# JinfengX/PointCloudPDF

Hardware: AMD Instinct MI355X
Metric: points/sec fwd+bwd (PT-v1 Seg50 + PDF U-decoder, 100k-pt scenes) (higher is better)
Workload: dtype f32

## Files before the change

### include/pdfops.h

```cpp
#ifndef PDFOPS_H
#define PDFOPS_H

#ifdef __cplusplus
extern "C" {
#endif

#define PDF_OK 0
#define PDF_ERR_BAD_ARG (-1)
#define PDF_ERR_NSAMPLE (-2)
#define PDF_ERR_UNSUPPORTED (-3)

#define PDF_ABI_VERSION 7
int pdf_abi_version(void);
const char *pdf_build_info(void);
int pdf_dist_fma_mode(void);
#define PDF_MMA_F32 0
#define PDF_MMA_F16 1
#define PDF_MMA_BF16 2

int pdf_knn_query(int m, int nsample, const float *xyz, const float *new_xyz,
                  const int *offset, const int *new_offset, int b,
                  int *idx, float *dist2, void *stream);

long pdf_knn_workspace_bytes(int b, int n, int m);
int pdf_knn_grid_supported(int nsample);
int pdf_knn_query_ws(int m, int nsample, int n, const float *xyz, const float *new_xyz, const int *offset,
                     const int *new_offset, int b, int *idx, float *dist2, void *workspace, long workspace_bytes,
                     void *stream);
int pdf_knn_grid_build(int n, const float *xyz, const int *offset, int b, void *workspace, long workspace_bytes, void *stream);
int pdf_knn_query_grid(int m, int nsample, int n, const float *xyz, const float *new_xyz, const int *offset, const int *new_offset, int b,
                       int *idx, float *dist2, void *workspace, long workspace_bytes, void *stream);
int pdf_knn_query_ws_counted(int m, int nsample, int n, const float *xyz, const float *new_xyz, const int *offset,
                             const int *new_offset, int b, int *idx, float *dist2, void *workspace, long workspace_bytes,
                             unsigned long long *pairs, void *stream);
int pdf_knn_query_list(int m, int nsample, const float *xyz, const float *new_xyz, const int *offset,
// ... 119 lines not shown
                      const float *k_points, float extent, float *weighted, void *stream);
int pdf_kpconv_scatter(int n, int m, int kp, int cin, const float *query, const float *support, const int *neighbors,
                       const float *grad_weighted, const float *k_points, float extent, float *grad_x, void *stream);
int pdf_rowlin_dgrad_bstats(long n, int k, int o, int nin, const float *const *x, long ldx, const float *const *w, float *y, long ldy,
                            const float *bx, long ldb, const float *bcoef, int brelu, float *partial, int *partial_rows,
                            int mma_input, void *stream);
int pdf_rowlin_forward_bn(long n, int k, int o, const float *x, long ldx, const float *w, const float *bias, const float *scale,
                          const float *shift, int relu, float *y, long ldy, float *partial, const float *gamma, const float *beta,
                          float *running_mean, float *running_var, float eps, float momentum, float *coef, int mma_input, void *stream);
int pdf_bn_act_backward_presummed(long n, int c, const float *gy, const float *x, const float *coef, int training, int relu,
                                  const float *partial, int partial_rows, float *sums, float *gx, void *stream);

int pdf_bn_coef_eval_or_partial(const float *partial, int rows, long n, int c, const float *gamma, const float *beta,
                                float *running_mean, float *running_var, int training, float eps, float momentum,
                                float *coef, void *stream);
int pdf_block_pre_forward(long n, int c, void *const *p, int training, float eps, float momentum, int mma_input, void *stream);
int pdf_block_pre_backward(long n, int c, void *const *p, int training, int mma_input, void *stream);
int pdf_block_post_forward(long n, int c, void *const *p, int training, float eps, float momentum, int mma_input, void *stream);
int pdf_block_post_backward(long n, int c, void *const *p, int training, int mma_input, void *stream);
int pdf_bottleneck_forward(long n, int nsample, int c, void *const *p, int training, float eps, float momentum, int storage_bf16, int mma_input, void *stream);
int pdf_bottleneck_backward(long n, int nsample, int c, void *const *p, int training, int entry_base, int storage_bf16, int mma_input, void *stream);
int pdf_linbn_forward(long n, int k, int o, void *const *p, int training, int relu, float eps, float momentum, int mma_input, void *stream);
int pdf_linbn_backward(long n, int k, int o, void *const *p, int training, int relu, int mma_input, void *stream);

int pdf_rowlin_forward_roww(long n, int k, int o, const float *x, long ldx, const float *w, int transpose_w, float *y, long ldy,
                            int accumulate, const float *roww, long rws, int mma_input, void *stream);
int pdf_rowlin_wgrad_roww(long n, int k, int o, const float *g, long ldg, const float *x, long ldx, float *dw, const float *roww,
                          long rws, float *ws, int mma_input, void *stream);
int pdf_bn_bwd_sums(long n, int c, const float *gy, const float *x, const float *coef, int relu, float *partial, float *sums,
                    void *stream);

int pdf_td_supported(int nsample, int cin, int cout);
int pdf_td_tables(long m, int b, const float *p_src, const float *p_new, const int *idx, const int *new_offset, float *rel4, float *Z,
                  float *scene_sums, long n, const int *inv_off, const int *inv_entry, int entry_base,
                  void *stream);
long pdf_td_gram_floats(int cin);
long pdf_td_fwd_scratch_floats(long n, int cin);
long pdf_td_bwd_scratch_floats(long m, int cin, int cout);
int pdf_td_forward(long n, long m, int cin, int cout, void *const *p, int training, float eps, float momentum, int mma_input, void *stream);
int pdf_td_backward(long n, long m, int cin, int cout, void *const *p, int entry_base, int mma_input, void *stream);

int pdf_seg_sum_rows(long n, int c, const float *src, const int *inv_off, const int *inv_entry, int entry_base, float scale, float *out,
                     void *stream);
int pdf_seg_sum_rows_own(long n, int c, int nsample, const float *src, const int *inv_off, const int *inv_entry, int entry_base, float scale,
                         const int *order, float *out, float *out_own, void *stream);
int pdf_seg_sum_rows_strided(long n, int c, const float *src, long src_stride, const int *inv_off, const int *inv_entry, int entry_base,
// ... 183 lines not shown
```

### pointcloudpdf_amd/_native.py

```python
import ctypes
import os
import threading

import torch

_HERE = os.path.dirname(os.path.abspath(__file__))
DIST_FMA = int(os.environ.get("PDFOPS_DIST_FMA", "0") or 0)
if DIST_FMA not in (0, 1, 2):
    raise RuntimeError(f"PDFOPS_DIST_FMA={DIST_FMA}: expected 0 (as written), 1 or 2 (csrc/pdfops_common.h)")


def library_path(dist_fma=0):
    return os.path.join(_HERE, "lib", "libpdfops.so" if not dist_fma else f"libpdfops_fma{int(dist_fma)}.so")


LIB_PATH = library_path(DIST_FMA)
ABI_VERSION = 7

c_int = ctypes.c_int
c_long = ctypes.c_long
c_void_p = ctypes.c_void_p
c_float = ctypes.c_float
c_double = ctypes.c_double

_PROTOS = {
    "knn_query": "iippppipp",
    "ball_query": "iiffppppipp",
    "random_ball_query": "iiffpppppipp",
    "farthest_point_sampling": "iippppp",
    "grouping_forward": "iiippp",
    "grouping_backward": "iiippp",
    "interpolation_forward": "iiipppp",
    "interpolation_backward": "iiipppp",
    "subtraction_forward": "iiipppp",
    "subtraction_backward": "iiipppp",
    "aggregation_forward": "iiiippppp",
    "aggregation_backward": "iiiipppppppp",
    "attention_relation_step_forward": "iiipppppp",
    "attention_relation_step_backward": "iiippppppppp",
    "attention_fusion_step_forward": "iiippppp",
# ... 581 lines not shown

        self.CopySeg = CopySeg
        lib.pdf_stage_copy.restype = c_int
        lib.pdf_stage_copy.argtypes = [c_int, c_void_p, c_void_p]
        lib.pdf_scene_morton_keys.restype = c_int
        lib.pdf_scene_morton_keys.argtypes = [c_long, c_int, c_void_p, c_void_p, c_void_p, c_void_p, c_void_p]
        lib.pdf_sgd_chunk.restype = c_int
        lib.pdf_sgd_chunk.argtypes = []
        lib.pdf_sgd_step.restype = c_int
        lib.pdf_sgd_step.argtypes = [c_int, c_void_p, c_void_p, ctypes.c_float, ctypes.c_float, ctypes.c_float, c_void_p, c_void_p]
        lib.pdf_grad_unscale.restype = c_int
        lib.pdf_grad_unscale.argtypes = [c_int, c_void_p, c_void_p, c_void_p, c_void_p, c_void_p]
        lib.pdf_scaler_update.restype = c_int
        lib.pdf_scaler_update.argtypes = [c_void_p, c_void_p, c_void_p, c_void_p, ctypes.c_float, ctypes.c_float, c_int, c_void_p]
        lib.pdf_adam_step.restype = c_int
        lib.pdf_adam_step.argtypes = [c_int, c_int, c_void_p, c_void_p, ctypes.c_double, ctypes.c_double, ctypes.c_double, ctypes.c_double,
                                      ctypes.c_double, c_int, c_void_p, c_void_p]
        lib.pdf_adam_grad_unscale.restype = c_int
        lib.pdf_adam_grad_unscale.argtypes = [c_int, c_void_p, c_void_p, c_void_p, c_void_p, c_void_p]
        lib.pdf_linbn_forward.restype = c_int
        lib.pdf_linbn_forward.argtypes = [c_long, c_int, c_int, c_void_p, c_int, c_int, ctypes.c_float, ctypes.c_float, c_int, c_void_p]
        lib.pdf_linbn_backward.restype = c_int
        lib.pdf_linbn_backward.argtypes = [c_long, c_int, c_int, c_void_p, c_int, c_int, c_int, c_void_p]
        lib.pdf_bottleneck_forward.restype = c_int
        lib.pdf_bottleneck_forward.argtypes = [c_long, c_int, c_int, c_void_p, c_int, ctypes.c_float, ctypes.c_float, c_int, c_int, c_void_p]
        lib.pdf_bottleneck_backward.restype = c_int
        lib.pdf_bottleneck_backward.argtypes = [c_long, c_int, c_int, c_void_p, c_int, c_int, c_int, c_int, c_void_p]
        for nm in ("pre_backward", "post_backward"):
            f = getattr(lib, "pdf_block_" + nm)
            f.restype = c_int
            f.argtypes = [c_long, c_int, c_void_p, c_int, c_int, c_void_p]
        lib.pdf_rowlin_multi.restype = c_int
        lib.pdf_rowlin_multi.argtypes = [c_long, c_int, c_int, c_int, c_int, c_void_p, c_long, c_void_p, c_int, c_void_p, c_void_p, c_void_p,
                                         c_int, c_void_p, c_long, c_int, c_int, c_void_p]
        lib.pdf_kpconv_supported.restype = c_int
        lib.pdf_kpconv_supported.argtypes = [c_int, c_int]
        for nm in ("pdf_kpconv_gather", "pdf_kpconv_scatter"):
            f = getattr(lib, nm)
            f.restype = c_int
            f.argtypes = [c_int, c_int, c_int, c_int, c_void_p, c_void_p, c_void_p, c_void_p, c_void_p, ctypes.c_float, c_void_p, c_void_p]
        lib.pdf_rowlin_wgrad_group.restype = c_int
        lib.pdf_rowlin_wgrad_group.argtypes = [c_long, c_int, c_int, c_int, c_void_p, c_long, c_void_p, c_long, c_void_p, c_void_p, c_void_p,
                                               c_void_p, c_void_p, c_void_p, c_int, c_void_p]
        lib.pdf_rowlin_wgrad_multi.restype = c_int
        lib.pdf_rowlin_wgrad_multi.argtypes = [c_long, c_int, c_int, c_int, c_void_p, c_long, c_void_p, c_long, c_void_p, c_void_p, c_int,
                                               c_void_p, c_void_p, c_void_p, c_int, c_void_p]
# ... 1026 lines not shown
```

### pointcloudpdf_amd/csrc/block.hip

```cpp
#include "pdfops_common.h"

namespace {
struct Err {
    int rc = 0;
    Err &operator<<(int r) { if (rc == 0 && r != 0) rc = r; return *this; }
};

}

extern "C" int pdf_bn_coef_eval_or_partial(const float *partial, int rows, long n, int c, const float *gamma, const float *beta,
                                           float *running_mean, float *running_var, int training, float eps, float momentum,
                                           float *coef, void *stream) {
    if (training) return pdf_bn_coef_from_partial(partial, rows, n, c, gamma, beta, running_mean, running_var, eps, momentum, coef, stream);
    return pdf_bn_coef(n, c, nullptr, gamma, beta, running_mean, running_var, 0, eps, momentum, coef, nullptr, stream);
}

extern "C" int pdf_block_pre_forward(long n, int c, void *const *p, int training, float eps, float momentum, int mma_input, void *stream) {
    if (n < 1 || !p) return PDF_ERR_BAD_ARG;
    if (!pdf_bn_supported(c)) return PDF_ERR_UNSUPPORTED;
    const float *x = (const float *)p[0], *W1 = (const float *)p[1], *g1 = (const float *)p[2], *b1 = (const float *)p[3];
    float *rm1 = (float *)p[4], *rv1 = (float *)p[5];
    float *z1 = (float *)p[12], *coef1 = (float *)p[13], *partial = (float *)p[17];
    Err e;
    if (training) {
// ... 180 lines not shown
    float *z = (float *)p[7], *coef = (float *)p[8], *partial = (float *)p[10];
    if (training) {
        e << pdf_rowlin_forward_bn(n, k, o, (const float *)p[0], k, (const float *)p[1], (const float *)p[2], nullptr, nullptr, 0, z, o, partial,
                                   (const float *)p[3], (const float *)p[4], (float *)p[5], (float *)p[6], eps, momentum, coef, mma_input, stream);
    } else {
        e << pdf_rowlin_forward(n, k, o, (const float *)p[0], k, (const float *)p[1], 0, (const float *)p[2], nullptr, nullptr, 0, z, o, 0, nullptr, mma_input, stream);
        e << pdf_bn_coef_eval_or_partial(partial, 0, n, o, (const float *)p[3], (const float *)p[4], (float *)p[5], (float *)p[6], 0, eps, momentum, coef, stream);
    }
    e << pdf_bn_apply(n, o, z, nullptr, coef, relu, (float *)p[9], stream);
    return e.rc;
}

extern "C" int pdf_linbn_backward(long n, int k, int o, void *const *p, int training, int relu, int mma_input, void *stream) {
    if (n < 1 || !p || !p[9]) return PDF_ERR_BAD_ARG;
    float *grads = (float *)p[6], *gz = (float *)p[7];
    const long ok = (long)o * k;
    Err e;
    e << pdf_bn_act_backward(n, o, (const float *)p[0], (const float *)p[2], nullptr, (const float *)p[3], training, relu, (float *)p[8],
                             grads + ok + o, gz, nullptr, stream);
    if (p[5]) e << pdf_rowlin_forward(n, o, k, gz, o, (const float *)p[4], 1, nullptr, nullptr, nullptr, 0, (float *)p[5], k, 0, nullptr, mma_input, stream);
    e << pdf_rowlin_wgrad(n, k, o, gz, o, (const float *)p[1], k, nullptr, nullptr, 0, grads, grads + ok, (float *)p[9], mma_input, stream);
    return e.rc;
}
```

### pointcloudpdf_amd/csrc/fused_layer.hip

```cpp
#include "fused_layer.h"
#include <algorithm>
#include <cstdlib>

namespace fl {

__host__ __device__ constexpr int tile_stride(int c) { return c / 8 > 32 ? 65 : 33; }
__host__ __device__ constexpr int aux_stride(int c) { return c / 8 <= 16 ? 17 : c / 8 + 1; }
constexpr int MAX_BLOCKS = 512;
static inline int env_blocks(const char *name, int dflt) {
    const char *v = getenv(name);
    const int x = v ? atoi(v) : 0;
    return x > 0 ? x : dflt;
}

struct WaveLds {
    float *tile;
    float *qtile;
    int *rowid;
    float *aux;
    int ts, as;
};

__device__ __forceinline__ void wave_sync() {
    __builtin_amdgcn_fence(__ATOMIC_RELEASE, "wavefront");
// ... 788 lines not shown
        for (int t = 0; t < RED_B; ++t) v[t] = src[(size_t)min(r + t * RED_RL, rows - 1) * stride];
#pragma unroll
        for (int t = 0; t < RED_B; ++t) v[t] = (r + t * RED_RL < rows) ? v[t] : 0.f;
#pragma unroll
        for (int t = 0; t < RED_B; t += 4) { s0 += (double)v[t]; s1 += (double)v[t + 1]; s2 += (double)v[t + 2]; s3 += (double)v[t + 3]; }
    }
    return (s0 + s1) + (s2 + s3);
}

__device__ __forceinline__ double wave_rows_sum(double v) {
    v += __shfl_xor(v, 16, 64);
    v += __shfl_xor(v, 32, 64);
    return v;
}
constexpr int RED_WAVES = RED_THREADS / 64;

struct BnpClosed {
    const double *mom;
    cfloat_p Wp1, bp1, sp, mean, rstd;
    double rows;
    int col_g;
    float *out4;
};
__global__ __launch_bounds__(RED_THREADS) void k_colsum(const float *__restrict__ partial, int rows, int width, int stride, float *__restrict__ out,
                                                        BnpClosed bc) {
    __shared__ double red[RED_WAVES][17];
    if (blockIdx.x * 16 >= (unsigned)width) {
        __shared__ double col[16];
        const int cl = threadIdx.x & 15, rl = threadIdx.x >> 4;
        const int c = cl < 6 ? cl : bc.col_g + (cl - 6);
        const double v = wave_rows_sum(cl < 15 ? strided_sum(partial + c, (size_t)stride, rl, rows) : 0.0);
        if ((threadIdx.x & 63) < 16) red[threadIdx.x >> 6][cl] = v;
        __syncthreads();
        if (threadIdx.x < 16) {
            double s = 0.0;
#pragma unroll
            for (int k = 0; k < RED_WAVES; ++k) s += red[k][threadIdx.x];
            col[threadIdx.x] = s;
        }
        __syncthreads();
        if (threadIdx.x < 12) {
            const double S[3] = {bc.mom[0], bc.mom[1], bc.mom[2]};
            const double M[3][3] = {{bc.mom[3], bc.mom[4], bc.mom[5]}, {bc.mom[4], bc.mom[6], bc.mom[7]}, {bc.mom[5], bc.mom[7], bc.mom[8]}};
            const int a = threadIdx.x < 3 ? (int)threadIdx.x : ((int)threadIdx.x - 3) / 3, b = threadIdx.x < 3 ? 0 : ((int)threadIdx.x - 3) % 3;
            const double w[3] = {(double)bc.Wp1[a * 3], (double)bc.Wp1[a * 3 + 1], (double)bc.Wp1[a * 3 + 2]};
            const double d = (double)bc.bp1[a] - (double)bc.mean[a], rs = (double)bc.rstd[a], sp = (double)bc.sp[a], R = bc.rows;
            const double s_a = col[a], u_a = col[3 + a];
            double r;
            if (threadIdx.x < 3) {
                const double sum_that = rs * (w[0] * S[0] + w[1] * S[1] + w[2] * S[2] + R * d);
                r = sp * (-(u_a / R) * sum_that);
            } else {
                const double T = rs * (w[0] * M[0][b] + w[1] * M[1][b] + w[2] * M[2][b] + d * S[b]);
                r = sp * (col[6 + 3 * a + b] - s_a * S[b] / R - u_a * T / R);
            }
            bc.out4[threadIdx.x] = (float)r;
        } else if (threadIdx.x < 16) {
            bc.out4[threadIdx.x] = 0.f;
        }
        return;
    }
    const int cl = threadIdx.x & 15, rl = threadIdx.x >> 4;
    const int col = blockIdx.x * 16 + cl;
    const double v = wave_rows_sum(col < width ? strided_sum(partial + col, (size_t)stride, rl, rows) : 0.0);
    if ((threadIdx.x & 63) < 16) red[threadIdx.x >> 6][cl] = v;
    __syncthreads();
    if (rl != 0 || col >= width) return;
    double s = 0.0;
#pragma unroll
    for (int k = 0; k < RED_WAVES; ++k) s += red[k][cl];
    out[col] = (float)s;
}

__global__ __launch_bounds__(RED_THREADS) void k_bn_finalize(const float *__restrict__ partial, int rows, int nch, double count,
                              const float *__restrict__ gamma, const float *__restrict__ beta, float eps, float momentum,
                              float *__restrict__ running_mean, float *__restrict__ running_var,
                              float *__restrict__ scale, float *__restrict__ shift, float *__restrict__ mean_out,
                              float *__restrict__ rstd_out) {
    __shared__ double red[2][RED_WAVES][17];
    const int cl = threadIdx.x & 15, rl = threadIdx.x >> 4;
    const int ch = blockIdx.x * 16 + cl;
    const double a = wave_rows_sum(ch < nch ? strided_sum(partial + ch, 2 * (size_t)nch, rl, rows) : 0.0);
    const double b = wave_rows_sum(ch < nch ? strided_sum(partial + nch + ch, 2 * (size_t)nch, rl, rows) : 0.0);
    if ((threadIdx.x & 63) < 16) { red[0][threadIdx.x >> 6][cl] = a; red[1][threadIdx.x >> 6][cl] = b; }
    __syncthreads();
    if (rl != 0 || ch >= nch) return;
    double s = 0.0, ss = 0.0;
#pragma unroll
    for (int k = 0; k < RED_WAVES; ++k) { s += red[0][k][cl]; ss += red[1][k][cl]; }
    const double mean = s / count;
    double var = ss / count - mean * mean;
    if (var < 0.0) var = 0.0;
    const float rstd = (float)(1.0 / sqrt(var + (double)eps));
    const float sc = gamma[ch] * rstd;
    scale[ch] = sc;
    shift[ch] = beta[ch] - (float)mean * sc;
    mean_out[ch] = (float)mean;
    rstd_out[ch] = rstd;
    if (running_mean) {
        const double unbiased = count > 1.0 ? var * count / (count - 1.0) : var;
        running_mean[ch] = (1.f - momentum) * running_mean[ch] + momentum * (float)mean;
        running_var[ch] = (1.f - momentum) * running_var[ch] + momentum * (float)unbiased;
    }
}

__global__ void k_bn_eval(int nch, const float *__restrict__ gamma, const float *__restrict__ beta, float eps,
                          const float *__restrict__ running_mean, const float *__restrict__ running_var,
                          float *__restrict__ scale, float *__restrict__ shift, float *__restrict__ mean_out,
                          float *__restrict__ rstd_out) {
    const int ch = blockIdx.x * blockDim.x + threadIdx.x;
    if (ch >= nch) return;
    const float rstd = 1.0f / sqrtf(running_var[ch] + eps);
    const float sc = gamma[ch] * rstd;
    scale[ch] = sc;
    shift[ch] = beta[ch] - running_mean[ch] * sc;
    if (mean_out) { mean_out[ch] = running_mean[ch]; rstd_out[ch] = rstd; }
}

void launch_bn_finalize(const float *partial, int rows, int nch, double count, const float *gamma, const float *beta, float eps,
                        float momentum, float *running_mean, float *running_var, float *scale, float *shift, float *mean_out,
                        float *rstd_out, hipStream_t s) {
    k_bn_finalize<<<pdf_divup(nch, 16), RED_THREADS, 0, s>>>(partial, rows, nch, count, gamma, beta, eps, momentum, running_mean, running_var,
                                                     scale, shift, mean_out, rstd_out);
}
void launch_bn_eval(int nch, const float *gamma, const float *beta, float eps, const float *running_mean, const float *running_var,
                    float *scale, float *shift, float *mean_out, float *rstd_out, hipStream_t s) {
    k_bn_eval<<<pdf_divup(nch, 64), 64, 0, s>>>(nch, gamma, beta, eps, running_mean, running_var, scale, shift, mean_out, rstd_out);
}
void launch_colsum(const float *partial, int rows, int width, float *out, hipStream_t s) {
    BnpClosed none;
    none.mom = nullptr; none.out4 = nullptr; none.rows = 0.0; none.col_g = 0;
    none.Wp1 = none.bp1 = none.sp = none.mean = none.rstd = as_const(nullptr);
    k_colsum<<<pdf_divup(width, 16), RED_THREADS, 0, s>>>(partial, rows, width, width, out, none);
}

template <typename KernelT>
static inline void allow_lds(KernelT kernel, size_t lds) {
    if (lds > 64 * 1024) (void)hipFuncSetAttribute(reinterpret_cast<const void *>(kernel), hipFuncAttributeMaxDynamicSharedMemorySize, (int)lds);
}

static inline int grid_for_points(long n, int cap) {
    static const int env_cap = env_blocks("PDFOPS_PT_BLOCKS_MFMA", 0);
    if (env_cap > 0) cap = env_cap;
    long g = (n + WPB - 1) / WPB;
    if (g > cap) g = cap;
    if (g < 1) g = 1;
    return (int)g;
}

enum Pass { P3 = 0, B1 = 1, B2 = 2, B3 = 3, P2 = 4 };
static inline int pass_grid(Pass pass, long n, int dflt_cap) {
    static const int env_cap[5] = {env_blocks("PDFOPS_PT_CAP_P3", 0), env_blocks("PDFOPS_PT_CAP_B1", 0), env_blocks("PDFOPS_PT_CAP_B2", 0),
                                   env_blocks("PDFOPS_PT_CAP_B3", 0), env_blocks("PDFOPS_PT_CAP_P2", 0)};
    return grid_for_points(n, env_cap[pass] > 0 ? env_cap[pass] : dflt_cap);
}

// ... 252 lines not shown
```

### pointcloudpdf_amd/dense.py

```python
import ctypes
import os
from ctypes import c_void_p

import torch

def _amp_fwd(fn):
    import functools

    from . import _native
    inner = torch.amp.custom_fwd(fn, device_type="cuda", cast_inputs=torch.float32)

    @functools.wraps(fn)
    def wrapped(ctx, *args, **kwargs):
        ctx._pdf_mma = _native.current_mma_input()
        return inner(ctx, *args, **kwargs)

    return wrapped


def _amp_bwd(fn):
    import functools

    from . import _native
    inner = torch.amp.custom_bwd(fn, device_type="cuda")
# ... 705 lines not shown

LINBN = True


def linbn_ok(lin, bn, x):
    if not LINBN:
        return False
    if not (x.is_cuda and x.dim() == 2 and x.dtype == torch.float32 and x.is_contiguous() and type(bn) is torch.nn.BatchNorm1d and bn.affine
            and bn.track_running_stats and bn.momentum is not None):
        return False
    k, o = lin.in_features, lin.out_features
    if k not in (32, 64, 128, 256, 512) or o % 16 or not _be().bn_supported(o):
        return False
    if torch.is_grad_enabled() and not bn.training and any(p.requires_grad for p in list(lin.parameters()) + list(bn.parameters())):
        return False
    return True


def linear_bn_act(lin, bn, x, relu):
    y = _LinBnFn.apply(lin, bn, relu, x, lin.weight, lin.bias, bn.weight, bn.bias)
    if bn.training:
        bump_counters([bn.num_batches_tracked])
    return y
```

### pointcloudpdf_amd/point_transformer.py

```python
import os

import torch

import torch.nn as nn
import torch.nn.functional as F

from . import _native, pointops
from . import dense
from .dense import _amp_bwd, _amp_fwd, bn_act as _bn_act, linear as _lin
from .geometry import Geometry, tag_of
from .registry import MODELS


def _seq(seq, x):
    mods = list(seq)
    i = 0
    while i < len(mods):
        m = mods[i]
        if (isinstance(m, nn.Linear) and i + 1 < len(mods) and isinstance(mods[i + 1], nn.BatchNorm1d) and x.dim() == 2
                and dense.linbn_ok(m, mods[i + 1], x)):
            relu = i + 2 < len(mods) and isinstance(mods[i + 2], nn.ReLU)
            x = dense.linear_bn_act(m, mods[i + 1], x, relu)
            i += 3 if relu else 2
            continue
        if isinstance(m, nn.Linear):
            x = _lin(m, x)
        elif isinstance(m, nn.BatchNorm1d) and type(m) is nn.BatchNorm1d and x.dim() == 2:
            relu = i + 1 < len(mods) and isinstance(mods[i + 1], nn.ReLU)
            x = _bn_act(m, x, None, relu)
            i += 1 if relu else 0
        else:
            x = m(x)
        i += 1
# ... 234 lines not shown
        else:
            self.linear1 = nn.Sequential(nn.Linear(out_planes, out_planes), nn.BatchNorm1d(out_planes), nn.ReLU(inplace=True))
            self.linear2 = nn.Sequential(nn.Linear(in_planes, out_planes), nn.BatchNorm1d(out_planes), nn.ReLU(inplace=True))

    @staticmethod
    def _scene_sizes(p, o):
        tag = tag_of(p)
        ends = tag[0].offset_host(tag[1]) if tag is not None else [int(v) for v in o.detach().cpu().tolist()]
        return [ends[0]] + [ends[i] - ends[i - 1] for i in range(1, len(ends))]

    def forward(self, pxo1, pxo2=None):
        if pxo2 is None:
            p, x, o = pxo1
            sizes = self._scene_sizes(p, o)
            means = _SceneMean.apply(x, o, sizes)
            ctx = _seq(self.linear2, means)
            tag = tag_of(p)
            sizes_dev = tag[0].sizes(tag[1]) if tag is not None else torch.diff(o.long(), prepend=o.new_zeros(1).long())
            rep = _RowsPerScene.apply(ctx, o, sizes_dev, sizes, x.shape[0])
            x = _seq(self.linear1, torch.cat((x, rep), 1))
        else:
            p1, x1, o1 = pxo1
            p2, x2, o2 = pxo2
            x = _seq(self.linear1, x1) + pointops.interpolation(p2, p1, _seq(self.linear2, x2), o2, o1)
        return x


class Bottleneck(nn.Module):

    expansion = 1

    def __init__(self, in_planes, planes, share_planes=8, nsample=16):
        super().__init__()
        self.linear1 = nn.Linear(in_planes, planes, bias=False)
        self.bn1 = nn.BatchNorm1d(planes)
        self.transformer = PointTransformerLayer(planes, planes, share_planes, nsample)
        self.bn2 = nn.BatchNorm1d(planes)
        self.linear3 = nn.Linear(planes, planes * self.expansion, bias=False)
        self.bn3 = nn.BatchNorm1d(planes * self.expansion)
        self.relu = nn.ReLU(inplace=True)

    def _apply(self, fn, *a, **kw):
        self.__dict__.pop("_pdf_params", None)
        return super()._apply(fn, *a, **kw)

    matrix_core = os.environ.get("PDFOPS_MATRIX_CORE", "1") != "0"
# ... 91 lines not shown
```

Measured before the change: 13.38 million.

## Fuse TransitionUp decoder branch into native forward/backward kernels

Adds a native fused TransitionUp path. Both Linear+BN+ReLU branches run through row-linear GEMMs, a single dual BN-finalize launch, and one combine kernel that applies BN, ReLU and 3-NN interpolation together. Backward adds a fused reduction, a colsum2 launch and an apply kernel, and groups the two weight-gradient GEMMs into one call when shapes match. The aim is fewer kernel launches and fewer intermediate tensor round-trips in the decoder, at the cost of extra code and an inverse-table build for the scatter backward.

```diff
diff --git a/include/pdfops.h b/include/pdfops.h
--- a/include/pdfops.h
+++ b/include/pdfops.h
@@ -10,7 +10,7 @@
 #define PDF_ERR_NSAMPLE (-2)
 #define PDF_ERR_UNSUPPORTED (-3)
 
-#define PDF_ABI_VERSION 7
+#define PDF_ABI_VERSION 8
 int pdf_abi_version(void);
 const char *pdf_build_info(void);
 int pdf_dist_fma_mode(void);
@@ -176,6 +176,11 @@
 int pdf_bottleneck_backward(long n, int nsample, int c, void *const *p, int training, int entry_base, int storage_bf16, int mma_input, void *stream);
 int pdf_linbn_forward(long n, int k, int o, void *const *p, int training, int relu, float eps, float momentum, int mma_input, void *stream);
 int pdf_linbn_backward(long n, int k, int o, void *const *p, int training, int relu, int mma_input, void *stream);
+int pdf_transition_up_supported(int k2, int c);
+long pdf_transition_up_partial_floats(long n1, long n2, int c);
+int pdf_transition_up_forward(long n1, long n2, int k2, int c, void *const *p, int training, float eps1, float momentum1, float eps2,
+                              float momentum2, int mma_input, void *stream);
+int pdf_transition_up_backward(long n1, long n2, int k2, int c, void *const *p, int entry_base, int mma_input, void *stream);
 
 int pdf_rowlin_forward_roww(long n, int k, int o, const float *x, long ldx, const float *w, int transpose_w, float *y, long ldy,
                             int accumulate, const float *roww, long rws, int mma_input, void *stream);
diff --git a/pointcloudpdf_amd/_native.py b/pointcloudpdf_amd/_native.py
--- a/pointcloudpdf_amd/_native.py
+++ b/pointcloudpdf_amd/_native.py
@@ -15,7 +15,7 @@
 
 
 LIB_PATH = library_path(DIST_FMA)
-ABI_VERSION = 7
+ABI_VERSION = 8
 
 c_int = ctypes.c_int
 c_long = ctypes.c_long
@@ -643,6 +643,15 @@
         lib.pdf_linbn_forward.argtypes = [c_long, c_int, c_int, c_void_p, c_int, c_int, ctypes.c_float, ctypes.c_float, c_int, c_void_p]
         lib.pdf_linbn_backward.restype = c_int
         lib.pdf_linbn_backward.argtypes = [c_long, c_int, c_int, c_void_p, c_int, c_int, c_int, c_void_p]
+        lib.pdf_transition_up_supported.restype = c_int
+        lib.pdf_transition_up_supported.argtypes = [c_int, c_int]
+        lib.pdf_transition_up_partial_floats.restype = c_long
+        lib.pdf_transition_up_partial_floats.argtypes = [c_long, c_long, c_int]
+        lib.pdf_transition_up_forward.restype = c_int
+        lib.pdf_transition_up_forward.argtypes = [c_long, c_long, c_int, c_int, c_void_p, c_int, ctypes.c_float, ctypes.c_float, ctypes.c_float,
+                                                  ctypes.c_float, c_int, c_void_p]
+        lib.pdf_transition_up_backward.restype = c_int
+        lib.pdf_transition_up_backward.argtypes = [c_long, c_long, c_int, c_int, c_void_p, c_int, c_int, c_void_p]
         lib.pdf_bottleneck_forward.restype = c_int
         lib.pdf_bottleneck_forward.argtypes = [c_long, c_int, c_int, c_void_p, c_int, ctypes.c_float, ctypes.c_float, c_int, c_int, c_void_p]
         lib.pdf_bottleneck_backward.restype = c_int
diff --git a/pointcloudpdf_amd/csrc/block.hip b/pointcloudpdf_amd/csrc/block.hip
--- a/pointcloudpdf_amd/csrc/block.hip
+++ b/pointcloudpdf_amd/csrc/block.hip
@@ -226,3 +226,97 @@
     e << pdf_rowlin_wgrad(n, k, o, gz, o, (const float *)p[1], k, nullptr, nullptr, 0, grads, grads + ok, (float *)p[9], mma_input, stream);
     return e.rc;
 }
+
+namespace fl {
+void launch_bn_finalize2(int nch, const float *partial0, int rows0, double count0, const float *gamma0, const float *beta0, float eps0,
+                         float momentum0, float *rm0, float *rv0, float *coef0, const float *partial1, int rows1, double count1,
+                         const float *gamma1, const float *beta1, float eps1, float momentum1, float *rm1, float *rv1, float *coef1, hipStream_t s);
+void launch_colsum2(const float *partial0, int rows0, float *out0, const float *partial1, int rows1, float *out1, int width, hipStream_t s);
+}
+long pdf_tup_bwd_partial_floats(long n1, long n2, int c);
+int pdf_tup_combine(long n1, int c, const float *z1, const float *z2, const int *idx, const float *weight, const int *order, const float *coef1,
+                    const float *coef2, float *out, void *stream);
+int pdf_tup_bwd_reduce(long n1, long n2, int c, const float *g, const float *z1, const float *coef1, const float *z2, const float *coef2,
+                       const float *weight, const int *inv_off, const int *inv_entry, int entry_base, const int *order2, float *gy2, float *partial,
+                       float **part1, float **part2, int *rows1, int *rows2, void *stream);
+int pdf_tup_bwd_apply(long n1, long n2, int c, const float *g, const float *z1, const float *coef1, const float *sums1, float *gz1, float *gy2,
+                      const float *z2, const float *coef2, const float *sums2, void *stream);
+
+static bool tup_fused() {
+    static const bool on = [] { const char *v = getenv("PDFOPS_TUP_FUSED"); return !(v && v[0] == '0'); }();
+    return on;
+}
+static long tup_fwd_rows1(long n1, int c) { return (pdf_rowlin_partial_floats(n1, c) + 63) / 64 * 64; }
+static bool tup_width(int k) { return k == 32 || k == 64 || k == 128 || k == 256 || k == 512; }
+
+extern "C" int pdf_transition_up_supported(int k2, int c) {
+    return tup_fused() && tup_width(k2) && tup_width(c) && c % 16 == 0 && pdf_bn_supported(c) ? 1 : 0;
+}
+extern "C" long pdf_transition_up_partial_floats(long n1, long n2, int c) {
+    if (n1 < 1 || n2 < 1 || c < 1) return 0;
+    const long fwd = tup_fwd_rows1(n1, c) + pdf_rowlin_partial_floats(n2, c), bwd = pdf_tup_bwd_partial_floats(n1, n2, c);
+    return fwd > bwd ? fwd : bwd;
+}
+
+extern "C" int pdf_transition_up_forward(long n1, long n2, int k2, int c, void *const *p, int training, float eps1, float momentum1, float eps2,
+                                         float momentum2, int mma_input, void *stream) {
+    if (n1 < 1 || n2 < 1 || !p) return PDF_ERR_BAD_ARG;
+    if (!tup_width(k2) || !tup_width(c) || !pdf_bn_supported(c)) return PDF_ERR_UNSUPPORTED;
+    for (int i = 0; i < 23; ++i) if (!p[i] && i != 2 && i != 9 && i != 16) return PDF_ERR_BAD_ARG;
+    float *z1 = (float *)p[17], *coef1 = (float *)p[18], *z2 = (float *)p[19], *coef2 = (float *)p[20];
+    float *part1 = (float *)p[22], *part2 = part1 + tup_fwd_rows1(n1, c);
+    hipStream_t s = static_cast<hipStream_t>(stream);
+    Err e;
+    e << pdf_rowlin_forward(n1, c, c, (const float *)p[0], c, (const float *)p[1], 0, (const float *)p[2], nullptr, nullptr, 0, z1, c, 0,
+                            training ? part1 : nullptr, mma_input, stream);
+    e << pdf_rowlin_forward(n2, k2, c, (const float *)p[7], k2, (const float *)p[8], 0, (const float *)p[9], nullptr, nullptr, 0, z2, c, 0,
+                            training ? part2 : nullptr, mma_input, stream);
+    if (e.rc) return e.rc;
+    if (training) {
+        fl::launch_bn_finalize2(c, part1, pdf_rowlin_partial_rows(n1, c, c), (double)n1, (const float *)p[3], (const float *)p[4], eps1, momentum1,
+                                (float *)p[5], (float *)p[6], coef1, part2, pdf_rowlin_partial_rows(n2, k2, c), (double)n2, (const float *)p[10],
+                                (const float *)p[11], eps2, momentum2, (float *)p[12], (float *)p[13], coef2, s);
+        e << pdf_launch_status();
+    } else {
+        e << pdf_bn_coef_eval_or_partial(nullptr, 0, n1, c, (const float *)p[3], (const float *)p[4], (float *)p[5], (float *)p[6], 0, eps1, momentum1, coef1, stream);
+        e << pdf_bn_coef_eval_or_partial(nullptr, 0, n2, c, (const float *)p[10], (const float *)p[11], (float *)p[12], (float *)p[13], 0, eps2, momentum2, coef2, stream);
+    }
+    e << pdf_tup_combine(n1, c, z1, z2, (const int *)p[14], (const float *)p[15], (const int *)p[16], coef1, coef2, (float *)p[21], stream);
+    return e.rc;
+}
+
+extern "C" int pdf_transition_up_backward(long n1, long n2, int k2, int c, void *const *p, int entry_base, int mma_input, void *stream) {
+    if (n1 < 1 || n2 < 1 || !p) return PDF_ERR_BAD_ARG;
+    if (!tup_width(k2) || !tup_width(c) || !pdf_bn_supported(c)) return PDF_ERR_UNSUPPORTED;
+    for (int i = 0; i < 21; ++i) if (!p[i] && i != 12 && i != 13 && i != 14) return PDF_ERR_BAD_ARG;
+    const float *g = (const float *)p[0], *x1 = (const float *)p[1], *z1 = (const float *)p[2], *coef1 = (const float *)p[3], *W1 = (const float *)p[4];
+    const float *x2 = (const float *)p[5], *z2 = (const float *)p[6], *coef2 = (const float *)p[7], *W2 = (const float *)p[8];
+    float *grads1 = (float *)p[15], *grads2 = (float *)p[16], *gz1 = (float *)p[17], *gz2 = (float *)p[18], *ws = (float *)p[20];
+    const long cc = (long)c * c, ck = (long)c * k2;
+    float *sums1 = grads1 + cc + c, *sums2 = grads2 + ck + c;
+    hipStream_t s = static_cast<hipStream_t>(stream);
+    Err e;
+    float *part1 = nullptr, *part2 = nullptr;
+    int rows1 = 0, rows2 = 0;
+    e << pdf_tup_bwd_reduce(n1, n2, c, g, z1, coef1, z2, coef2, (const float *)p[9], (const int *)p[10], (const int *)p[11], entry_base,
+                            (const int *)p[12], gz2, (float *)p[19], &part1, &part2, &rows1, &rows2, stream);
+    if (e.rc) return e.rc;
+    fl::launch_colsum2(part1, rows1, sums1, part2, rows2, sums2, 2 * c, s);
+    e << pdf_launch_status();
+    e << pdf_tup_bwd_apply(n1, n2, c, g, z1, coef1, sums1, gz1, gz2, z2, coef2, sums2, stream);
+    if (p[13]) e << pdf_rowlin_forward(n1, c, c, gz1, c, W1, 1, nullptr, nullptr, nullptr, 0, (float *)p[13], c, 0, nullptr, mma_input, stream);
+    if (p[14]) e << pdf_rowlin_forward(n2, c, k2, gz2, c, W2, 1, nullptr, nullptr, nullptr, 0, (float *)p[14], k2, 0, nullptr, mma_input, stream);
+    bool grouped = false;
+    if (n1 == n2 && k2 == c) {
+        const float *gs[2] = {gz1, gz2}, *xs[2] = {x1, x2}, *none[2] = {nullptr, nullptr};
+        const int relu[2] = {0, 0};
+        float *dw[2] = {grads1, grads2}, *db[2] = {grads1 + cc, grads2 + ck};
+        const int rc = pdf_rowlin_wgrad_group(n1, c, c, 2, gs, c, xs, c, none, none, relu, dw, db, ws, mma_input, stream);
+        if (rc != PDF_ERR_UNSUPPORTED) { e << rc; grouped = true; }
+    }
+    if (!grouped) {
+        e << pdf_rowlin_wgrad(n1, c, c, gz1, c, x1, c, nullptr, nullptr, 0, grads1, grads1 + cc, ws, mma_input, stream);
+        e << pdf_rowlin_wgrad(n2, k2, c, gz2, c, x2, k2, nullptr, nullptr, 0, grads2, grads2 + ck, ws, mma_input, stream);
+    }
+    return e.rc;
+}
diff --git a/pointcloudpdf_amd/csrc/fused_layer.hip b/pointcloudpdf_amd/csrc/fused_layer.hip
--- a/pointcloudpdf_amd/csrc/fused_layer.hip
+++ b/pointcloudpdf_amd/csrc/fused_layer.hip
@@ -834,6 +834,19 @@
     int col_g;
     float *out4;
 };
+__device__ __forceinline__ void colsum_block(int blk, const float *__restrict__ partial, int rows, int width, int stride, float *__restrict__ out,
+                                             double (*red)[17]) {
+    const int cl = threadIdx.x & 15, rl = threadIdx.x >> 4;
+    const int col = blk * 16 + cl;
+    const double v = wave_rows_sum(col < width ? strided_sum(partial + col, (size_t)stride, rl, rows) : 0.0);
+    if ((threadIdx.x & 63) < 16) red[threadIdx.x >> 6][cl] = v;
+    __syncthreads();
+    if (rl != 0 || col >= width) return;
+    double s = 0.0;
+#pragma unroll
+    for (int k = 0; k < RED_WAVES; ++k) s += red[k][cl];
+    out[col] = (float)s;
+}
 __global__ __launch_bounds__(RED_THREADS) void k_colsum(const float *__restrict__ partial, int rows, int width, int stride, float *__restrict__ out,
                                                         BnpClosed bc) {
     __shared__ double red[RED_WAVES][17];
@@ -872,48 +885,62 @@
         }
         return;
     }
+    colsum_block(blockIdx.x, partial, rows, width, stride, out, red);
+}
+
+struct ColsumSet { const float *partial; int rows, width; float *out; };
+__global__ __launch_bounds__(RED_THREADS) void k_colsum2(ColsumSet a, ColsumSet b, int blocks0) {
+    __shared__ double red[RED_WAVES][17];
+    const bool first = (int)blockIdx.x < blocks0;
+    const ColsumSet d = first ? a : b;
+    colsum_block(first ? blockIdx.x : blockIdx.x - blocks0, d.partial, d.rows, d.width, d.width, d.out, red);
+}
+
+struct BnFinalize {
+    const float *partial; int rows; double count;
+    const float *gamma, *beta; float eps, momentum;
+    float *running_mean, *running_var, *scale, *shift, *mean_out, *rstd_out;
+};
+__device__ __forceinline__ void bn_finalize_block(int blk, int nch, const BnFinalize &d, double (*red)[RED_WAVES][17]) {
     const int cl = threadIdx.x & 15, rl = threadIdx.x >> 4;
-    const int col = blockIdx.x * 16 + cl;
-    const double v = wave_rows_sum(col < width ? strided_sum(partial + col, (size_t)stride, rl, rows) : 0.0);
-    if ((threadIdx.x & 63) < 16) red[threadIdx.x >> 6][cl] = v;
+    const int ch = blk * 16 + cl;
+    const double a = wave_rows_sum(ch < nch ? strided_sum(d.partial + ch, 2 * (size_t)nch, rl, d.rows) : 0.0);
+    const double b = wave_rows_sum(ch < nch ? strided_sum(d.partial + nch + ch, 2 * (size_t)nch, rl, d.rows) : 0.0);
+    if ((threadIdx.x & 63) < 16) { red[0][threadIdx.x >> 6][cl] = a; red[1][threadIdx.x >> 6][cl] = b; }
     __syncthreads();
-    if (rl != 0 || col >= width) return;
-    double s = 0.0;
-#pragma unroll
-    for (int k = 0; k < RED_WAVES; ++k) s += red[k][cl];
-    out[col] = (float)s;
-}
-
+    if (rl != 0 || ch >= nch) return;
+    double s = 0.0, ss = 0.0;
+#pragma unroll
+    for (int k = 0; k < RED_WAVES; ++k) { s += red[0][k][cl]; ss += red[1][k][cl]; }
+    const double mean = s / d.count;
+    double var = ss / d.count - mean * mean;
+    if (var < 0.0) var = 0.0;
+    const float rstd = (float)(1.0 / sqrt(var + (double)d.eps));
+    const float sc = d.gamma[ch] * rstd;
+    d.scale[ch] = sc;
+    d.shift[ch] = d.beta[ch] - (float)mean * sc;
+    d.mean_out[ch] = (float)mean;
+    d.rstd_out[ch] = rstd;
+    if (d.running_mean) {
+        const double unbiased = d.count > 1.0 ? var * d.count / (d.count - 1.0) : var;
+        d.running_mean[ch] = (1.f - d.momentum) * d.running_mean[ch] + d.momentum * (float)mean;
+        d.running_var[ch] = (1.f - d.momentum) * d.running_var[ch] + d.momentum * (float)unbiased;
+    }
+}
 __global__ __launch_bounds__(RED_THREADS) void k_bn_finalize(const float *__restrict__ partial, int rows, int nch, double count,
                               const float *__restrict__ gamma, const float *__restrict__ beta, float eps, float momentum,
                               float *__restrict__ running_mean, float *__restrict__ running_var,
                               float *__restrict__ scale, float *__restrict__ shift, float *__restrict__ mean_out,
                               float *__restrict__ rstd_out) {
     __shared__ double red[2][RED_WAVES][17];
-    const int cl = threadIdx.x & 15, rl = threadIdx.x >> 4;
-    const int ch = blockIdx.x * 16 + cl;
-    const double a = wave_rows_sum(ch < nch ? strided_sum(partial + ch, 2 * (size_t)nch, rl, rows) : 0.0);
-    const double b = wave_rows_sum(ch < nch ? strided_sum(partial + nch + ch, 2 * (size_t)nch, rl, rows) : 0.0);
-    if ((threadIdx.x & 63) < 16) { red[0][threadIdx.x >> 6][cl] = a; red[1][threadIdx.x >> 6][cl] = b; }
-    __syncthreads();
-    if (rl != 0 || ch >= nch) return;
-    double s = 0.0, ss = 0.0;
-#pragma unroll
-    for (int k = 0; k < RED_WAVES; ++k) { s += red[0][k][cl]; ss += red[1][k][cl]; }
-    const double mean = s / count;
-    double var = ss / count - mean * mean;
-    if (var < 0.0) var = 0.0;
-    const float rstd = (float)(1.0 / sqrt(var + (double)eps));
-    const float sc = gamma[ch] * rstd;
-    scale[ch] = sc;
-    shift[ch] = beta[ch] - (float)mean * sc;
-    mean_out[ch] = (float)mean;
-    rstd_out[ch] = rstd;
-    if (running_mean) {
-        const double unbiased = count > 1.0 ? var * count / (count - 1.0) : var;
-        running_mean[ch] = (1.f - momentum) * running_mean[ch] + momentum * (float)mean;
-        running_var[ch] = (1.f - momentum) * running_var[ch] + momentum * (float)unbiased;
-    }
+    const BnFinalize d = {partial, rows, count, gamma, beta, eps, momentum, running_mean, running_var, scale, shift, mean_out, rstd_out};
+    bn_finalize_block(blockIdx.x, nch, d, red);
+}
+__global__ __launch_bounds__(RED_THREADS) void k_bn_finalize2(int nch, BnFinalize d0, BnFinalize d1) {
+    __shared__ double red[2][RED_WAVES][17];
+    const int per = (nch + 15) / 16;
+    const bool first = (int)blockIdx.x < per;
+    bn_finalize_block(first ? blockIdx.x : blockIdx.x - per, nch, first ? d0 : d1, red);
 }
 
 __global__ void k_bn_eval(int nch, const float *__restrict__ gamma, const float *__restrict__ beta, float eps,
@@ -944,6 +971,18 @@
     none.mom = nullptr; none.out4 = nullptr; none.rows = 0.0; none.col_g = 0;
     none.Wp1 = none.bp1 = none.sp = none.mean = none.rstd = as_const(nullptr);
     k_colsum<<<pdf_divup(width, 16), RED_THREADS, 0, s>>>(partial, rows, width, width, out, none);
+}
+
+void launch_bn_finalize2(int nch, const float *partial0, int rows0, double count0, const float *gamma0, const float *beta0, float eps0,
+                         float momentum0, float *rm0, float *rv0, float *coef0, const float *partial1, int rows1, double count1,
+                         const float *gamma1, const float *beta1, float eps1, float momentum1, float *rm1, float *rv1, float *coef1, hipStream_t s) {
+    const BnFinalize d0 = {partial0, rows0, count0, gamma0, beta0, eps0, momentum0, rm0, rv0, coef0, coef0 + nch, coef0 + 2 * nch, coef0 + 3 * nch};
+    const BnFinalize d1 = {partial1, rows1, count1, gamma1, beta1, eps1, momentum1, rm1, rv1, coef1, coef1 + nch, coef1 + 2 * nch, coef1 + 3 * nch};
+    k_bn_finalize2<<<2 * pdf_divup(nch, 16), RED_THREADS, 0, s>>>(nch, d0, d1);
+}
+void launch_colsum2(const float *partial0, int rows0, float *out0, const float *partial1, int rows1, float *out1, int width, hipStream_t s) {
+    const ColsumSet a = {partial0, rows0, width, out0}, b = {partial1, rows1, width, out1};
+    k_colsum2<<<2 * pdf_divup(width, 16), RED_THREADS, 0, s>>>(a, b, pdf_divup(width, 16));
 }
 
 template <typename KernelT>
diff --git a/pointcloudpdf_amd/csrc/transition_up.hip b/pointcloudpdf_amd/csrc/transition_up.hip
--- /dev/null
+++ b/pointcloudpdf_amd/csrc/transition_up.hip
@@ -0,0 +1,227 @@
+#include "pdfops_common.h"
+
+namespace tu {
+
+constexpr int TB = 256;
+constexpr int SB = 8;
+typedef float v4f __attribute__((ext_vector_type(4)));
+
+struct FastDiv { unsigned d, m, s; };
+static inline FastDiv mk_fastdiv(unsigned d) {
+    FastDiv f; f.d = d;
+    if (d == 1) { f.m = 0; f.s = 0; return f; }
+    unsigned s = 0;
+    while ((1u << s) < d) ++s;
+    f.s = s;
+    f.m = (unsigned)(((1ull << (32 + s)) + d - 1) / d - (1ull << 32));
+    return f;
+}
+__device__ __forceinline__ unsigned fdiv(unsigned x, FastDiv f) {
+    if (f.d == 1) return x;
+    const unsigned t = __umulhi(x, f.m);
+    return (t + ((x - t) >> 1)) >> (f.s - 1);
+}
+__device__ __forceinline__ v4f relu4(v4f v) { return __builtin_elementwise_max(v, (v4f)(0.f)); }
+
+__global__ __launch_bounds__(TB) void k_combine(unsigned total, FastDiv cvd, const int *__restrict__ order, const v4f *__restrict__ z1,
+                                                const v4f *__restrict__ z2, const int *__restrict__ idx, const float *__restrict__ weight,
+                                                const v4f *__restrict__ coef1, const v4f *__restrict__ coef2, v4f *__restrict__ out) {
+    const unsigned cv = cvd.d, blk = pdf_xcd_chunked_block(blockIdx.x, gridDim.x);
+    const unsigned w = blk * TB + threadIdx.x;
+    if (w >= total) return;
+    const unsigned sq = fdiv(w, cvd), col = w - sq * cv, r = order ? (unsigned)order[sq] : sq;
+    int j[3]; float wt[3]; v4f v[3];
+#pragma unroll
+    for (int i = 0; i < 3; ++i) { j[i] = idx[(unsigned long)r * 3 + i]; wt[i] = weight[(unsigned long)r * 3 + i]; }
+    const v4f a = z1[(unsigned long)r * cv + col];
+#pragma unroll
+    for (int i = 0; i < 3; ++i) v[i] = z2[(unsigned long)max(j[i], 0) * cv + col];
+    const v4f s1 = coef1[col], t1 = coef1[cv + col], s2 = coef2[col], t2 = coef2[cv + col];
+    v4f acc = (v4f)(0.f);
+#pragma unroll
+    for (int i = 0; i < 3; ++i) acc += (j[i] >= 0 ? relu4(v[i] * s2 + t2) : (v4f)(0.f)) * wt[i];
+    __builtin_nontemporal_store(relu4(a * s1 + t1) + acc, out + (unsigned long)r * cv + col);
+}
+
+static inline int fine_groups(long n, int c) {
+    const long rpb = (long)TB * 4 / c, per = n * c >= (1L << 22) ? 8 : 4;
+    const long g = (n + rpb * per - 1) / (rpb * per);
+    return (int)(g > 1024 ? 1024 : (g < 1 ? 1 : g));
+}
+static inline long coarse_rows_per_group(long n, int c) {
+    const long rpb = (long)TB * 4 / c;
+    const long per = (n + rpb * 2048 - 1) / (rpb * 2048);
+    return rpb * (per < 1 ? 1 : per);
+}
+static inline int coarse_groups(long n, int c) {
+    const long r = coarse_rows_per_group(n, c);
+    return (int)((n + r - 1) / r);
+}
+
+struct ReduceArgs {
+    int g1;
+    long n1, n2, rows2;
+    int c;
+    const float *g, *z1, *coef1;
+    const float *z2, *coef2;
+    const float *w;
+    const int *inv_off, *inv_entry, *order2;
+    int entry_base;
+    float *gy2;
+    float *part1, *part2;
+};
+
+__global__ __launch_bounds__(TB) void k_bwd_reduce(ReduceArgs A) {
+    extern __shared__ float red[];
+    const int c = A.c, tpr = c / 4, rpb = TB / tpr;
+    const int tr = threadIdx.x / tpr, tc = threadIdx.x % tpr;
+    const bool fine = (int)blockIdx.x < A.g1;
+    const float *coef = fine ? A.coef1 : A.coef2;
+    float s[4] = {0.f, 0.f, 0.f, 0.f}, sx[4] = {0.f, 0.f, 0.f, 0.f};
+    float sc[4], sh[4], mu[4], rs[4];
+#pragma unroll
+    for (int k = 0; k < 4; ++k) { sc[k] = coef[tc * 4 + k]; sh[k] = coef[c + tc * 4 + k]; mu[k] = coef[2 * c + tc * 4 + k]; rs[k] = coef[3 * c + tc * 4 + k]; }
+    if (fine) {
+        for (long r = (long)blockIdx.x * rpb + tr; r < A.n1; r += (long)A.g1 * rpb) {
+            const float4 g4 = *reinterpret_cast<const float4 *>(A.g + r * c + tc * 4);
+            const float4 x4 = *reinterpret_cast<const float4 *>(A.z1 + r * c + tc * 4);
+            const float g[4] = {g4.x, g4.y, g4.z, g4.w}, xv[4] = {x4.x, x4.y, x4.z, x4.w};
+#pragma unroll
+            for (int k = 0; k < 4; ++k) {
+                const float gm = xv[k] * sc[k] + sh[k] > 0.f ? g[k] : 0.f;
+                s[k] += gm;
+                sx[k] += gm * ((xv[k] - mu[k]) * rs[k]);
+            }
+        }
+    } else {
+        const long b = (long)blockIdx.x - A.g1, first = b * A.rows2, last = min(first + A.rows2, A.n2);
+        for (long pos = first + tr; pos < last; pos += rpb) {
+            const long v = A.order2 ? (long)A.order2[pos] : pos;
+            int t = A.inv_off[v];
+            const int end = A.inv_off[v + 1];
+            const float4 x4 = *reinterpret_cast<const float4 *>(A.z2 + v * c + tc * 4);
+            float4 a0 = make_float4(0.f, 0.f, 0.f, 0.f), a1 = a0;
+            for (; t < end; t += SB) {
+                unsigned e[SB];
+                float4 x[SB];
+                float ww[SB];
+#pragma unroll
+                for (int k = 0; k < SB; ++k) e[k] = (unsigned)(A.inv_entry[min(t + k, end - 1)] - A.entry_base);
+#pragma unroll
+                for (int k = 0; k < SB; ++k) { x[k] = *reinterpret_cast<const float4 *>(A.g + (size_t)(e[k] / 3u) * c + tc * 4); ww[k] = A.w[e[k]]; }
+#pragma unroll
+                for (int k = 0; k < SB; ++k) {
+                    const float wk = t + k < end ? ww[k] : 0.f;
+                    float4 &a = (k & 1) ? a1 : a0;
+                    a.x += x[k].x * wk; a.y += x[k].y * wk; a.z += x[k].z * wk; a.w += x[k].w * wk;
+                }
+            }
+            a0.x += a1.x; a0.y += a1.y; a0.z += a1.z; a0.w += a1.w;
+            *reinterpret_cast<float4 *>(A.gy2 + v * c + tc * 4) = a0;
+            const float g[4] = {a0.x, a0.y, a0.z, a0.w}, xv[4] = {x4.x, x4.y, x4.z, x4.w};
+#pragma unroll
+            for (int k = 0; k < 4; ++k) {
+                const float gm = xv[k] * sc[k] + sh[k] > 0.f ? g[k] : 0.f;
+                s[k] += gm;
+                sx[k] += gm * ((xv[k] - mu[k]) * rs[k]);
+            }
+        }
+    }
+#pragma unroll
+    for (int k = 0; k < 4; ++k) { red[threadIdx.x * 8 + k] = s[k]; red[threadIdx.x * 8 + 4 + k] = sx[k]; }
+    __syncthreads();
+    if ((int)threadIdx.x < tpr) {
+        float *partial = fine ? A.part1 + (size_t)blockIdx.x * 2 * c : A.part2 + (size_t)(blockIdx.x - A.g1) * 2 * c;
+#pragma unroll
+        for (int k = 0; k < 8; ++k) {
+            float a = 0.f;
+            for (int rr = 0; rr < rpb; ++rr) a += red[(rr * tpr + threadIdx.x) * 8 + k];
+            const int ch = threadIdx.x * 4 + (k & 3);
+            partial[k < 4 ? ch : c + ch] = a;
+        }
+    }
+}
+
+struct ApplyArgs {
+    int blocks1;
+    long n4a, n4b;
+    int c4;
+    const float4 *g, *z1, *coef1, *sums1;
+    float4 *gz1;
+    float4 *gy2;
+    const float4 *z2, *coef2, *sums2;
+    float inv_n1, inv_n2;
+};
+__global__ __launch_bounds__(TB) void k_bwd_apply(ApplyArgs A) {
+    const bool first = (int)blockIdx.x < A.blocks1;
+    const float4 *gy = first ? A.g : A.gy2, *x = first ? A.z1 : A.z2, *coef = first ? A.coef1 : A.coef2, *sums = first ? A.sums1 : A.sums2;
+    float4 *gx = first ? A.gz1 : A.gy2;
+    const long n4 = first ? A.n4a : A.n4b;
+    const float inv_n = first ? A.inv_n1 : A.inv_n2;
+    const long blk = first ? blockIdx.x : blockIdx.x - A.blocks1, nblk = first ? A.blocks1 : (long)gridDim.x - A.blocks1;
+    const int c4 = A.c4;
+    for (long e = blk * TB + threadIdx.x; e < n4; e += nblk * TB) {
+        const int cc = (int)(e % c4);
+        const float4 g4 = gy[e], x4 = x[e], sc = coef[cc], sh = coef[c4 + cc], mu = coef[2 * c4 + cc], rs = coef[3 * c4 + cc];
+        const float4 s1 = sums[cc], s2 = sums[c4 + cc];
+        float4 o;
+#define TU_ONE(f)                                                         \
+        {                                                                 \
+            const float gm = x4.f * sc.f + sh.f > 0.f ? g4.f : 0.f;       \
+            const float xh = (x4.f - mu.f) * rs.f;                        \
+            o.f = sc.f * (gm - s1.f * inv_n - xh * s2.f * inv_n);         \
+        }
+        TU_ONE(x) TU_ONE(y) TU_ONE(z) TU_ONE(w)
+#undef TU_ONE
+        gx[e] = o;
+    }
+}
+
+static inline int grid_elems(long n4) {
+    const long g = (n4 + TB - 1) / TB;
+    return (int)(g > 2048 ? 2048 : (g < 1 ? 1 : g));
+}
+
+}
+
+long pdf_tup_bwd_partial_floats(long n1, long n2, int c) { return ((long)tu::fine_groups(n1, c) + tu::coarse_groups(n2, c)) * 2 * c; }
+
+int pdf_tup_combine(long n1, int c, const float *z1, const float *z2, const int *idx, const float *weight, const int *order, const float *coef1,
+                    const float *coef2, float *out, void *stream) {
+    if ((long)n1 * (c / 4) >= (1L << 31) || n1 * 3 >= (1L << 31)) return PDF_ERR_UNSUPPORTED;
+    const unsigned total = (unsigned)(n1 * (c / 4));
+    tu::k_combine<<<(total + tu::TB - 1) / tu::TB, tu::TB, 0, static_cast<hipStream_t>(stream)>>>(
+        total, tu::mk_fastdiv((unsigned)(c / 4)), order, reinterpret_cast<const tu::v4f *>(z1), reinterpret_cast<const tu::v4f *>(z2), idx, weight,
+        reinterpret_cast<const tu::v4f *>(coef1), reinterpret_cast<const tu::v4f *>(coef2), reinterpret_cast<tu::v4f *>(out));
+    return pdf_launch_status();
+}
+
+int pdf_tup_bwd_reduce(long n1, long n2, int c, const float *g, const float *z1, const float *coef1, const float *z2, const float *coef2,
+                       const float *weight, const int *inv_off, const int *inv_entry, int entry_base, const int *order2, float *gy2, float *partial,
+                       float **part1, float **part2, int *rows1, int *rows2, void *stream) {
+    if (n1 * 3 >= (1L << 31)) return PDF_ERR_UNSUPPORTED;
+    tu::ReduceArgs A;
+    A.g1 = tu::fine_groups(n1, c);
+    const int g2 = tu::coarse_groups(n2, c);
+    A.n1 = n1; A.n2 = n2; A.rows2 = tu::coarse_rows_per_group(n2, c); A.c = c;
+    A.g = g; A.z1 = z1; A.coef1 = coef1; A.z2 = z2; A.coef2 = coef2; A.w = weight;
+    A.inv_off = inv_off; A.inv_entry = inv_entry; A.order2 = order2; A.entry_base = entry_base;
+    A.gy2 = gy2; A.part1 = partial; A.part2 = partial + (size_t)A.g1 * 2 * c;
+    *part1 = A.part1; *part2 = A.part2; *rows1 = A.g1; *rows2 = g2;
+    tu::k_bwd_reduce<<<A.g1 + g2, tu::TB, tu::TB * 8 * sizeof(float), static_cast<hipStream_t>(stream)>>>(A);
+    return pdf_launch_status();
+}
+
+int pdf_tup_bwd_apply(long n1, long n2, int c, const float *g, const float *z1, const float *coef1, const float *sums1, float *gz1, float *gy2,
+                      const float *z2, const float *coef2, const float *sums2, void *stream) {
+    tu::ApplyArgs A;
+    A.n4a = n1 * (c / 4); A.n4b = n2 * (c / 4); A.c4 = c / 4;
+    A.blocks1 = tu::grid_elems(A.n4a);
+#define F4(p) reinterpret_cast<const float4 *>(p)
+    A.g = F4(g); A.z1 = F4(z1); A.coef1 = F4(coef1); A.sums1 = F4(sums1); A.z2 = F4(z2); A.coef2 = F4(coef2); A.sums2 = F4(sums2);
+#undef F4
+    A.gz1 = reinterpret_cast<float4 *>(gz1); A.gy2 = reinterpret_cast<float4 *>(gy2);
+    A.inv_n1 = (float)(1.0 / (double)n1); A.inv_n2 = (float)(1.0 / (double)n2);
+    tu::k_bwd_apply<<<A.blocks1 + tu::grid_elems(A.n4b), tu::TB, 0, static_cast<hipStream_t>(stream)>>>(A);
+    return pdf_launch_status();
+}
diff --git a/pointcloudpdf_amd/dense.py b/pointcloudpdf_amd/dense.py
--- a/pointcloudpdf_amd/dense.py
+++ b/pointcloudpdf_amd/dense.py
@@ -751,3 +751,99 @@
     if bn.training:
         bump_counters([bn.num_batches_tracked])
     return y
+
+
+class _TransitionUpFn(torch.autograd.Function):
+    @staticmethod
+    @_amp_fwd
+    def forward(ctx, bn1, bn2, idx, weight, x1, x2, W1, b1, gamma1, beta1, W2, b2, gamma2, beta2):
+        from . import _native
+        be = _be()
+        _rcd(x1, x2, idx, weight, W1, W2, gamma1, gamma2)
+        lib = be.lib
+        n1, c = x1.shape
+        n2, k2 = x2.shape
+        training = bn1.training
+        e = lambda *shape: torch.empty(shape, dtype=torch.float32, device=x1.device)
+        z1, coef1, z2, coef2, out = e(n1, c), e(4 * c), e(n2, c), e(4 * c), e(n1, c)
+        partial = e(int(lib.pdf_transition_up_partial_floats(n1, n2, c)))
+        order = _native.order_of(idx)
+        opt = lambda t: t.data_ptr() if t is not None else None
+        ptrs = [x1.data_ptr(), W1.data_ptr(), opt(b1), gamma1.data_ptr(), beta1.data_ptr(), bn1.running_mean.data_ptr(), bn1.running_var.data_ptr(),
+                x2.data_ptr(), W2.data_ptr(), opt(b2), gamma2.data_ptr(), beta2.data_ptr(), bn2.running_mean.data_ptr(), bn2.running_var.data_ptr(),
+                idx.data_ptr(), weight.data_ptr(), opt(order), z1.data_ptr(), coef1.data_ptr(), z2.data_ptr(), coef2.data_ptr(), out.data_ptr(),
+                partial.data_ptr()]
+        rc = lib.pdf_transition_up_forward(n1, n2, k2, c, (c_void_p * len(ptrs))(*ptrs), int(training), ctypes.c_float(bn1.eps),
+                                           ctypes.c_float(bn1.momentum), ctypes.c_float(bn2.eps), ctypes.c_float(bn2.momentum), _mma(), be._stream())
+        if rc != 0:
+            raise RuntimeError(f"pdf_transition_up_forward failed with status {rc}")
+        ctx.save_for_backward(x1, x2, z1, z2, coef1, coef2, W1, W2, idx, weight)
+        ctx.cfg = (training, b1 is not None, b2 is not None)
+        return out
+
+    @staticmethod
+    @_amp_bwd
+    def backward(ctx, g):
+        from . import _native
+        x1, x2, z1, z2, coef1, coef2, W1, W2, idx, weight = ctx.saved_tensors
+        training, has_b1, has_b2 = ctx.cfg
+        if not training:
+            raise RuntimeError("fused TransitionUp: backward is implemented for training mode (batch statistics)")
+        be = _be()
+        lib = be.lib
+        n1, c = x1.shape
+        n2, k2 = x2.shape
+        e = lambda *shape: torch.empty(shape, dtype=torch.float32, device=x1.device)
+        need1, need2 = ctx.needs_input_grad[4], ctx.needs_input_grad[5]
+        gx1, gx2 = e(n1, c) if need1 else None, e(n2, k2) if need2 else None
+        cc, ck = c * c, c * k2
+        grads1, grads2, gz1, gz2 = e(cc + 3 * c), e(ck + 3 * c), e(n1, c), e(n2, c)
+        partial = e(int(lib.pdf_transition_up_partial_floats(n1, n2, c)))
+        g = g.contiguous()
+        wsf = max(int(lib.pdf_rowlin_wgrad_ws_floats(n1, c, c, 1)), int(lib.pdf_rowlin_wgrad_ws_floats(n2, k2, c, 1)),
+                  int(lib.pdf_rowlin_wgrad_ws_floats(n1, c, c, 2)) if (n1 == n2 and k2 == c) else 0, 1)
+        ws = e(wsf)
+        inv_off, inv_entry, entry_base = _native.inverse_table(idx, n2)
+        order2 = _native.src_order_of(idx, n2)
+        opt = lambda t: t.data_ptr() if t is not None else None
+        ptrs = [g.data_ptr(), x1.data_ptr(), z1.data_ptr(), coef1.data_ptr(), W1.data_ptr(), x2.data_ptr(), z2.data_ptr(), coef2.data_ptr(),
+                W2.data_ptr(), weight.data_ptr(), inv_off.data_ptr(), inv_entry.data_ptr(), opt(order2), opt(gx1), opt(gx2), grads1.data_ptr(),
+                grads2.data_ptr(), gz1.data_ptr(), gz2.data_ptr(), partial.data_ptr(), ws.data_ptr()]
+        rc = lib.pdf_transition_up_backward(n1, n2, k2, c, (c_void_p * len(ptrs))(*ptrs), int(entry_base), _mma(), be._stream())
+        if rc != 0:
+            raise RuntimeError(f"pdf_transition_up_backward failed with status {rc}")
+        return (None, None, None, None, gx1, gx2,
+                grads1[:cc].view(c, c), grads1[cc:cc + c] if has_b1 else None, grads1[cc + 2 * c:cc + 3 * c], grads1[cc + c:cc + 2 * c],
+                grads2[:ck].view(c, k2), grads2[ck:ck + c] if has_b2 else None, grads2[ck + 2 * c:ck + 3 * c], grads2[ck + c:ck + 2 * c])
+
+
+TUP = True
+
+
+def transition_up_ok(mod, x1, x2):
+    if not TUP:
+        return False
+    l1, l2 = list(mod.linear1), list(mod.linear2)
+    if not (len(l1) == 3 and len(l2) == 3 and all(type(s[0]) is nn.Linear and type(s[1]) is nn.BatchNorm1d and isinstance(s[2], nn.ReLU) for s in (l1, l2))):
+        return False
+    for (lin, bn), x in (((l1[0], l1[1]), x1), ((l2[0], l2[1]), x2)):
+        if not (x.is_cuda and x.dim() == 2 and x.dtype == torch.float32 and x.is_contiguous() and bn.affine and bn.track_running_stats
+                and bn.momentum is not None and x.shape[1] == lin.in_features and x.shape[0] >= 1):
+            return False
+    c, k2 = l1[0].out_features, l2[0].in_features
+    if l1[0].in_features != c or l2[0].out_features != c or l1[1].training != l2[1].training:
+        return False
+    if not _be().lib.pdf_transition_up_supported(k2, c):
+        return False
+    params = [p for s in (l1, l2) for m in s[:2] for p in m.parameters()]
+    if torch.is_grad_enabled() and not l1[1].training and (x1.requires_grad or x2.requires_grad or any(p.requires_grad for p in params)):
+        return False
+    return True
+
+
+def transition_up(mod, idx, weight, x1, x2):
+    lin1, bn1, lin2, bn2 = mod.linear1[0], mod.linear1[1], mod.linear2[0], mod.linear2[1]
+    out = _TransitionUpFn.apply(bn1, bn2, idx, weight, x1, x2, lin1.weight, lin1.bias, bn1.weight, bn1.bias, lin2.weight, lin2.bias, bn2.weight, bn2.bias)
+    if bn1.training:
+        bump_counters([bn1.num_batches_tracked, bn2.num_batches_tracked])
+    return out
diff --git a/pointcloudpdf_amd/point_transformer.py b/pointcloudpdf_amd/point_transformer.py
--- a/pointcloudpdf_amd/point_transformer.py
+++ b/pointcloudpdf_amd/point_transformer.py
@@ -9,6 +9,7 @@
 from . import dense
 from .dense import _amp_bwd, _amp_fwd, bn_act as _bn_act, linear as _lin
 from .geometry import Geometry, tag_of
+from .pointops._ops import _interp_tables
 from .registry import MODELS
 
 
@@ -289,6 +290,10 @@
         else:
             p1, x1, o1 = pxo1
             p2, x2, o2 = pxo2
+            if dense.transition_up_ok(self, x1, x2):
+                idx, weight = _interp_tables(p2, p1, o2, o1, 3)
+                if idx.shape == (x1.shape[0], 3) and idx.dtype == torch.int32 and idx.is_contiguous() and weight.is_contiguous():
+                    return dense.transition_up(self, idx, weight, x1, x2)
             x = _seq(self.linear1, x1) + pointops.interpolation(p2, p1, _seq(self.linear2, x2), o2, o1)
         return x
 
```

Measured after the change: 13.75 million, median of 6. 2.8% higher.
